# yxlllc/DDSP-SVC

Measured on AMD Instinct MI355X. Metric: audio samples/sec, CombSub 44.1kHz 256-harm hop512, higher is better.
Workload: dtype f32; 1 GPU; combsub B=32/GPU x 10 s utterances (F=862, T=441344), n_mag 256/256/256, sr 44100, hop 512, DSP path (HOT-1 + HOT-2) from resident f0 / raw controls ~N(0,1) / uniform noise, signal only; batch_per_gpu=32, frames=862, samples_per_utterance=441344, parallelism=utterance-shard x1

## Files before the change

ddsp_svc_amd/_ffi.py:

```python
import ctypes
import os
import threading

import torch

from . import build as _build

c_int, c_long, c_float, c_double, c_size_t = (ctypes.c_int, ctypes.c_long, ctypes.c_float,
                                              ctypes.c_double, ctypes.c_size_t)
P = ctypes.c_void_p

SIGNATURES = {
    "ddsp_hip_version": (c_int, []),
    "ddsp_hip_error_string": (ctypes.c_char_p, [c_int]),
    "ddsp_hip_set_tuning": (c_int, [ctypes.c_char_p, c_long]),
    "ddsp_hip_get_tuning": (c_long, [ctypes.c_char_p]),
    "ddsp_hip_window_impulse_response": (c_int, [P, c_int, P, c_long, c_int, P, P]),
    "ddsp_hip_upsample": (c_int, [P, c_int, c_int, c_int, c_int, P, P]),
    "ddsp_hip_remove_above_fmax": (c_int, [P, P, c_long, c_int, c_float, c_int, P, P]),
    "ddsp_hip_phase": (c_int, [P, P, c_int, c_int, c_int, c_double, c_int, P, P, P, P, P]),
    "ddsp_hip_ir_table_bytes": (c_size_t, [c_int]),
    "ddsp_hip_ir_table": (c_int, [c_int, P, P]),
    "ddsp_hip_allpass_response": (c_int, [P, c_long, c_long, c_int, P, P, P]),
    "ddsp_hip_impulse_response": (c_int, [P, c_long, P, c_long, c_int, c_float, c_int, P, c_long, c_int, P, P, P]),
# ... 3 lines not shown
    "ddsp_hip_allpass_backward": (c_int, [P, c_long, c_long, c_int, P, P, P, P]),
    "ddsp_hip_allpass_taps_backward": (c_int, [P, P, c_long, c_long, c_int, P, P, P, P, P]),
    "ddsp_hip_fft_convolve": (c_int, [P, c_int, P, P, P, P, c_int, c_int, c_int, c_int, c_int, P]),
    "ddsp_hip_frequency_filter_workspace_bytes": (c_size_t, [c_int, c_int, c_int]),
    "ddsp_hip_frequency_filter": (c_int, [P, P, c_long, P, c_long, c_int, P, c_int, c_int, c_int, c_int, P, P, P,
                                          c_size_t, P]),
    "ddsp_hip_fft_convolve_backward": (c_int, [P, c_int, P, P, P, P, c_int, c_int, c_int, c_int, P]),
    "ddsp_hip_sins_synth": (c_int, [P, P, P, P, c_long, P, c_long, P, c_long, P, c_int,
                                    c_int, c_int, c_int, c_double, c_int, c_int, c_int, c_int,
                                    P, P, P, P, P, P, c_size_t, c_int, P, P, ctypes.c_ulonglong, ctypes.c_ulonglong]),
    "ddsp_hip_combsub_synth": (c_int, [P, P, P, P, c_long, P, c_long, P, c_long, P, c_int,
                                       c_int, c_int, c_int, c_double, c_int, c_int, c_int, c_int,
                                       P, P, P, P, P, P, P, c_size_t, c_int, P, P, ctypes.c_ulonglong, ctypes.c_ulonglong]),
    "ddsp_hip_uniform_noise": (c_int, [ctypes.c_ulonglong, ctypes.c_ulonglong, c_int, c_long, P, P]),
    "ddsp_hip_synth_workspace_bytes": (c_size_t, [c_int, c_int, c_int, c_int]),
    "ddsp_hip_tail_layout": (c_int, [c_int, c_int, c_int, c_int, c_int, c_int, c_int, c_int, c_int, P]),
    "ddsp_hip_combsub_tail_backward_ws_bytes": (c_size_t, [c_int, c_int, c_int, c_int]),
    "ddsp_hip_combsub_tail_backward": (c_int, [P, P, c_long, P, c_long, P, c_long, P, c_int, P, P, P, c_int, c_int, c_int, c_double,
                                               c_int, P, P, P, P, P, c_size_t, P]),
    "ddsp_hip_combtooth": (c_int, [P, P, P, c_int, c_int, c_int, c_double, c_int, P, P]),
    "ddsp_hip_sinusoid_bank": (c_int, [P, P, P, P, c_long, c_int, c_int, c_int, c_int, c_double, c_int, P, P]),
    "ddsp_hip_sinusoid_bank_backward_scratch_bytes": (c_size_t, [c_int, c_int, c_int]),
    "ddsp_hip_sinusoid_bank_backward": (c_int, [P, P, P, P, c_long, P, c_int, c_int, c_int, c_int, c_double, c_int,
                                                P, P, P]),
    "ddsp_hip_fast_source": (c_int, [P, c_int, c_int, c_int, c_double, P, P, P, P]),
    "ddsp_hip_stft_filter": (c_int, [P, P, c_int, P, c_long, P, c_long, P, c_long, P, c_long, c_float, P, c_int,
                                     c_int, c_int, c_int, c_int, c_int, P, P]),
    "ddsp_hip_stft_filter_backward": (c_int, [P, P, c_int, P, c_long, P, c_long, P, c_long, P, c_long, c_float, P,
                                              c_int, c_int, c_int, P, c_int, c_int, c_int, P, P, P, P, P]),
    "ddsp_hip_combsubfast_synth": (c_int, [P, P, P, P, c_long, P, c_long, P, c_long, P, c_int, P,
# ... 177 lines not shown
```

ddsp_svc_amd/csrc/api.hip:

```cpp
#include "../../include/ddsp_hip.h"
#include "kernels.h"
#include "philox.h"
#include "splice.h"
#include "resample.h"
#include "frame_features.h"
#include "resblock.h"
#include "generator_tail.h"
#include <atomic>
#include <stdio.h>
#include <mutex>
#include <vector>
#include <stdlib.h>
#include <string.h>

using namespace ddsp;

namespace ddsp {
thread_local int t_geometry_batch = 0;
namespace {
const char* const kKnobNames[KNOB_COUNT] = {"BLK_WPS", "BLK_RUN", "BLK_PADLDS", "FFT_RUN", "STFT_WPS", "STFT_RUN",
                                            "MEL_WPS", "MEL_RUN", "FIR_MAX_SLOTS", "SINS_V1", "TAPS_GEMM", "STREAM_LAYOUT",
                                            "BLK_TURNS", "CZT_ROUNDS", "CZT_TURNS", "SINS_NOSKIP", "SMALL_PATH", "LANE_ROWS", "LANES", "FIR_BWD_DIRECT", "BWD_WPS", "TAPS_FULL",
                                            "AP_BWD_SPLIT", "SINS_SEQ", "BATCH_SPLIT"};
std::atomic<long> g_knobs[KNOB_COUNT];
std::once_flag g_knobs_once;
bool knob_is_inert(int i, long v) {
#ifdef DDSP_AB_GENERATIONS
  (void)i; (void)v;
  return false;
#else
  if (v == 0) return false;
  return i == KNOB_BLK_WPS || i == KNOB_BLK_PADLDS || (i == KNOB_SINS_V1 && v == 2);
#endif
}
void knobs_from_env() {
  for (int i = 0; i < KNOB_COUNT; ++i) {
    char name[64] = "DDSP_HIP_";
    strncat(name, kKnobNames[i], sizeof(name) - strlen(name) - 1);
// ... 48 lines not shown
  bool ok;
  Carver(void* p, size_t n) : base(static_cast<char*>(p)), size(n), used(0), ok(p != nullptr || n == 0) {}
  template <class T> T* take(size_t count) {
    size_t off = align_up(used, 256);
    size_t end = off + count * sizeof(T);
    if (end > size) { ok = false; used = end; return nullptr; }
    used = end;
    return reinterpret_cast<T*>(base + off);
  }
};

struct SynthWs {
  float *buf0, *buf1, *taps, *re, *im;
  float *taps_nz, *nzbuf;
  float *taps3;
};

struct BranchEvents {
  hipEvent_t fork = nullptr, join = nullptr, mid[2] = {nullptr, nullptr};
};

template <class T>
struct DevicePool {
  std::mutex m;
  std::vector<T*> idle[64];
  T* take(int dev) {
    std::lock_guard<std::mutex> lock(m);
    if (idle[dev].empty()) return nullptr;
    T* t = idle[dev].back();
    idle[dev].pop_back();
// ... 177 lines not shown
size_t carve_synth(Carver& c, int B, int F, int hop, int n_max, SynthWs& w) {
  const size_t BT = (size_t)B * F * hop, R = (size_t)B * F, N = 2 * (size_t)(n_max - 1);
  w.buf0 = c.take<float>(BT);
  w.buf1 = c.take<float>(BT);
  w.taps = c.take<float>(R * N);
  if (2 * R * n_max <= BT) {
    w.re = w.buf0;
    w.im = w.buf0 + R * n_max;
  } else {
    w.re = c.take<float>(R * n_max);
    w.im = c.take<float>(R * n_max);
  }
  w.taps_nz = c.take<float>(R * N);
  w.nzbuf = c.take<float>(BT);
  w.taps3 = ((long)R < kSmallRows || (n_max == 256 && hop == 512 && !fused_off())) ? c.take<float>(R * N) : nullptr;
  return align_up(c.used, 256);
}

}

extern "C" {

int ddsp_hip_version(void) { return DDSP_HIP_VERSION; }

const char* ddsp_hip_error_string(int code) {
  switch (code) {
    case 0: return "success";
    case DDSP_HIP_EINVAL: return "ddsp_hip: invalid argument (null pointer or non-positive size)";
    case DDSP_HIP_EHOP: return "ddsp_hip: hop > 2048 is not supported by the phase scan";
    case DDSP_HIP_ESHAPE: return "ddsp_hip: shape not supported by the requested kernel";
    case DDSP_HIP_EWS: return "ddsp_hip: workspace too small";
// ... 336 lines not shown
  const bool all256 = n_ap == 256 && n_harm == 256 && n_nz == 256 && !t_taps_gemm;
  float* nz = a.noise_out ? a.noise_out : w.nzbuf;
  if (w.taps3 && fused_shape_ok(R, F, hop, n_ap, n_harm, n_nz, a.fir_impl, a.gen.on != 0, true)) {
    ExciterJob exc;
    if (make_exciter_job(a.f0_frames, a.initial_phase, B, F, hop, a.sr, a.infer, a.phase0, w.buf0, &exc) != 0) return DDSP_HIP_EHOP;
    TapsJobs jobs;
    jobs.n = 0;
    const int half = taps_half_ok(F, hop, a.fir_impl) ? 1 : 0;
    int ok = launch_taps_pfa510(a.c2, a.ld2, nullptr, 0, 0, DDSP_HIP_ACT_EXP, 1.0f / 128.0f, a.t2, DDSP_HIP_MODE_HANN, nullptr, R,
                                n_nz, w.taps_nz, st, 0.f, &jobs, half);
    ok |= launch_taps_pfa510(a.c0, a.ld0, nullptr, 0, 1, DDSP_HIP_ACT_NONE, 1.0f, a.t0, DDSP_HIP_MODE_ROLL, nullptr, R, n_ap,
                             w.taps, st, 0.f, &jobs);
    ok |= launch_taps_pfa510(a.c1, a.ld1, nullptr, 0, 0, DDSP_HIP_ACT_EXP, 1.0f, a.t1, DDSP_HIP_MODE_DYNAMIC, a.f0_frames, R,
                             n_harm, w.taps3, st, (float)a.sr, &jobs);
    if (ok != 0 || launch_taps_pfa510_batch(jobs, st, &exc) != 0) return DDSP_HIP_ESHAPE;
    const FirSecond second{a.noise, a.noise_is_u01, w.taps_nz, nullptr, nz, nullptr, half};
    if (launch_fir_blk(w.buf0, 0, w.taps, nullptr, w.buf1, nullptr, B, F, hop, 2 * (n_ap - 1), st, a.gen.on ? &a.gen : nullptr, &second) < 0)
      return DDSP_HIP_ESHAPE;
    if (launch_fir(w.buf1, 0, w.taps3, nz, a.signal, a.harmonic, B, F, hop, 2 * (n_harm - 1), a.fir_impl, st) < 0)
      return DDSP_HIP_ESHAPE;
    return 0;
  }
  Branch br(st, aux_stream);
  long layout = knob(KNOB_STREAM_LAYOUT);
  if (layout != 1) layout = 4;
  if (!all256) layout = 1;
  int rc = 0;
  if (layout == 4) {
    rc = launch_combtooth(a.f0_frames, a.initial_phase, B, F, hop, a.sr, a.infer, a.phase0, w.buf0, br.aux);
    br.publish(0);
// ... 21 lines not shown

}

extern "C" {

size_t ddsp_hip_synth_workspace_bytes(int B, int F, int hop, int n_max) {
  if (B <= 0 || F <= 0 || hop <= 0 || n_max < 2) return 0;
  Carver c(nullptr, (size_t)-1);
  c.base = nullptr;
  SynthWs w;
  const LanePlan p = lane_plan(B, F);
  if (p.nsub == 1) return carve_synth(c, B, F, hop, n_max, w);
  size_t end = 0;
  for (int l = 0; l < p.slots; ++l) end = carve_synth(c, p.Bs, F, hop, n_max, w);
  return end;
}

int ddsp_hip_tail_layout(int combsub, int B, int F, int hop, int n0, int n1, int n2, int fir_impl, int in_kernel_noise,
                         long long offsets[6]) {
  if (!offsets || B <= 0 || F <= 0 || hop <= 0) return DDSP_HIP_EINVAL;
  for (int i = 0; i < 6; ++i) offsets[i] = -1;
  const TapsFormScope form;
  int n_max = n1 > n2 ? n1 : n2;
  if (combsub && n0 > n_max) n_max = n0;
  if (lane_plan(B, F).nsub > 1) return 0;
  if (!fused_shape_ok((long)B * F, F, hop, n0, n1, n2, fir_impl, in_kernel_noise != 0, combsub != 0)) return 0;
  constexpr uintptr_t kBase = 4096;
  Carver c(reinterpret_cast<void*>(kBase), (size_t)1 << 60);
  SynthWs w;
  carve_synth(c, B, F, hop, n_max, w);
// ... 143 lines not shown
  if (gen.on && !(hop == 512 && n_nz <= 257 && (fir_impl == 0 || fir_impl == 5))) return DDSP_HIP_ESHAPE;
  int n_max = n_ap > n_nz ? n_ap : n_nz;
  if (n_harm > n_max) n_max = n_harm;
  hipStream_t st = S(stream);
  const TapsFormScope form;
  const TailCall call{f0_frames, initial_phase, phase0, c_gd, ld_gd, c_harm, ld_harm, c_nz, ld_nz, noise, noise_is_u01,
                      B, F, hop, sr, infer, n_ap, n_harm, n_nz, table_ap, table_harm, table_nz, signal, harmonic_or_null,
                      noise_out_or_null, fir_impl, gen};
  const LanePlan plan = lane_plan(B, F);
  if (plan.nsub > 1) {
    const int rc = run_lanes(call, plan, ws, ws_bytes, n_max, st, aux_stream, combsub_rows);
    return rc != 0 ? rc : finish();
  }
  Carver c(ws, ws_bytes);
  SynthWs w;
  carve_synth(c, B, F, hop, n_max, w);
  if (!c.ok) return DDSP_HIP_EWS;
  const int rc = combsub_rows(call, w, st, aux_stream);
  return rc != 0 ? rc : finish();
}

size_t ddsp_hip_stft_workspace_bytes(int B, int F, int hop) {
  if (B <= 0 || F <= 0 || hop <= 0) return 0;
  return align_up((size_t)B * F * hop * sizeof(float), 256);
}

int ddsp_hip_fast_source(const float* f0_frames, int B, int F, int hop, double sr, float* rad_acc, float* phase_frames,
                         float* combtooth, void* stream) {
  if (B < 0 || F <= 0 || hop <= 0 || !(sr > 0)) return DDSP_HIP_EINVAL;
  if (B == 0) return 0;
  if (!f0_frames || !rad_acc) return DDSP_HIP_EINVAL;
  if (launch_fast_source(f0_frames, B, F, hop, sr, rad_acc, phase_frames, combtooth, S(stream)) != 0)
// ... 473 lines not shown
```

ddsp_svc_amd/csrc/fir_blk.hip:

```cpp
#include "fft_1024p.h"
#include "kernels.h"
#include "philox.h"
#include <stdlib.h>
#include <type_traits>

namespace ddsp {

using fft::cmul;

constexpr int FB_HOP = 512;

#ifdef DDSP_HIP_TIMELINE
__device__ long long* g_blk_timeline = nullptr;
__global__ void k_set_blk_timeline(long long* p) { g_blk_timeline = p; }
#define BLK_STAMP(slot) do { if (g_blk_timeline && threadIdx.x == 0 && (slot) < 32) g_blk_timeline[(long)blockIdx.x * 32 + (slot)] = (long long)wall_clock64(); } while (0)
#define BLK_STAMP_CYC(slot) do { if (g_blk_timeline && threadIdx.x == 0 && (slot) < 32) g_blk_timeline[(long)blockIdx.x * 32 + (slot)] = (long long)__builtin_readcyclecounter(); } while (0)
#define BLK_STAMP_WHERE(slot) do { if (g_blk_timeline && threadIdx.x == 0) g_blk_timeline[(long)blockIdx.x * 32 + (slot)] = ((long long)__builtin_amdgcn_s_getreg(0xF814) << 32) | (unsigned)__builtin_amdgcn_s_getreg(0xF804); } while (0)
#else
#define BLK_STAMP(slot) do { } while (0)
#define BLK_STAMP_CYC(slot) do { } while (0)
#define BLK_STAMP_WHERE(slot) do { } while (0)
#endif

struct FirBlkGeom {
// ... 222 lines not shown
    if (stamp_it) BLK_STAMP_CYC(29);
    BLK_STAMP(3 + q - q_first);
  }
}
#endif

struct FirJob {
  const float* x; int x_is_u01;
  const float* taps; const float* addend;
  float* out; float* out_plain;
  int rng;
  int taps_half;
};
struct FirJobs { FirJob j[2]; };

template <bool RNG = false, bool SEQ = false>
#ifndef DDSP_FIR_NT
#define DDSP_FIR_NT 11
#endif
#if DDSP_FIR_NT & 1
#define FB_LD_X ld_nt
#else
#define FB_LD_X ld
#endif
#if DDSP_FIR_NT & 2
#define FB_LD_T ld_nt
#else
#define FB_LD_T ld
#endif
#if DDSP_FIR_NT & 4
#define FB_ST st_nt
#else
#define FB_ST st
#endif
#if DDSP_FIR_NT & 8
#define FB_LD_A ld_nt
#else
#define FB_LD_A ld
#endif
__global__ void __launch_bounds__(128, 3) k_fir_blk6(FirJobs jobs, FirBlkGeom g, NoiseGen rng) {
  int jb = SEQ ? 0 : (int)blockIdx.y;
seq_next:
 {
  const FirJob& J = jobs.j[jb];
  const float* __restrict__ x = J.x;
  const int x_is_u01 = J.x_is_u01;
  const bool draw = RNG && J.rng != 0;
  const float* __restrict__ taps = J.taps;
  const float* __restrict__ addend = J.addend;
  float* __restrict__ out = J.out;
  float* __restrict__ out_plain = J.out_plain;
  using PL = fft::Plan1024P;
  constexpr int NF = PL::N, P = PL::P, S = 8;
  __shared__ __attribute__((aligned(16))) f32x2 ex[3][PL::WORDS];
  f32x2* const bX = ex[0];
  f32x2* const bY = ex[1];
  f32x2* const bC = ex[2];
  const int tid = threadIdx.x;
  const int b = blockIdx.x / g.runs_per_utt;
// ... 111 lines not shown
      if (m == 0) bm = own_mirror ? B0 : bm;
      a[m] = fft::add_conj(bm, a[m]);
    }
  };

  const int bw = 2 * q_first - 1;
  TapRow t1 = load_taps(bw > 0 ? bw : 0), t2 = load_taps(bw + 1);
  Blk x0 = load_blk(bw >= 0 ? bw : g.F), x1 = x0;
  typename PL::Tw tw;
  tw.init(tid);
  typename PL::Ix ix;
  ix.init(tid);
  f32x2 Hc[S];
#pragma unroll
  for (int m = 0; m < S; ++m) Hc[m] = f32x2{0.f, 0.f};
  const bool has_add = addend != nullptr, has_plain = out_plain != nullptr;
  const int turn = __builtin_amdgcn_s_getreg(0x1804) & 1;
  const int turns_mask = g.turns ? 1 : 0;
  float add[S];
#pragma unroll
  for (int i = 0; i < S; ++i) add[i] = 0.f;
  for (int q = q_first - 1; q < q_last; ++q) {
    const bool warm = q < q_first;
    if ((q + turn) & turns_mask) __builtin_amdgcn_s_setprio(1);
    else __builtin_amdgcn_s_setprio(0);
    const int b0 = 2 * q;
    f32x2 z0[S], z1[S];
#if defined(DDSP_B6_HALF_PASS_AHEAD)
    if (warm) pack_taps(t1, t2, z0);
    else pack_blk(x0, b0 < g.F, z0);
    t1 = load_taps(b0 + 3);
    t2 = load_taps(b0 + 4);
    PL::template forward_s<true, true>(z0, tw, bX, bY, ix);
// ... 22 lines not shown
#endif
    if (warm) {
      park(z0, bC);
      __syncthreads();
#pragma unroll
      for (int m = 0; m < S; ++m) z0[m] = f32x2{0.f, 0.f};
    }
    f32x2 B0;
    split_and_products(z0, z1, Hc, bC, bX, B0);
    __syncthreads();
    hermitian(z0, bX, B0);
#if defined(DDSP_B6_HALF_PASS_AHEAD)
    x0 = load_blk(b0 + 2);
    x1 = load_blk(b0 + 3);
#endif
    const int e0 = b0 * FB_HOP - 256 + tid;
    const int off_a = b0 > 0 ? 4 * e0 : BufF32::kOutOfRange;
    const int off_b = 4 * e0 + 8 * P;
    auto t_off = [&](int i) -> int { return i < 2 ? off_a + 4 * P * i : off_b + 4 * P * (i - 2); };
#if defined(DDSP_B6_HALF_PASS_AHEAD)
    if (has_add && !warm) {
#pragma unroll
      for (int i = 0; i < S; ++i) add[i] = add_buf.FB_LD_A(t_off(i));
    }
#endif
    f32x2 zt[S];
    pack_taps(t1, t2, zt);
#if !defined(DDSP_B6_HALF_PASS_AHEAD)
    t1 = load_taps(b0 + 5, pass_after);
    t2 = load_taps(b0 + 6, pass_after);
// ... 10 lines not shown
      }
#pragma unroll
      for (int i = 0; i < S; ++i) out_buf.FB_ST(fmaf(sg, d[i], add[i]), t_off(i));
      if (q == g.pairs - 1) {
#pragma unroll
        for (int m = 4; m < S; ++m) {
          const int off = t_off(4 + m);
          const float v = nsg * z0[m].y;
          if (has_plain) plain_buf.FB_ST(v, off);
          out_buf.FB_ST(v + (has_add ? add_buf.FB_LD_A(off) : 0.f), off);
        }
      }
    }
#pragma unroll
    for (int m = 0; m < 4; ++m) tail[m] = z0[4 + m].y;
#if !defined(DDSP_B6_HALF_PASS_AHEAD)
    if (has_add && q + 1 < q_last) {
      const int n0 = e0 + 2 * FB_HOP;
      const int nx_a = b0 + 2 > 0 ? 4 * n0 : BufF32::kOutOfRange, nx_b = 4 * n0 + 8 * P;
#pragma unroll
      for (int i = 0; i < S; ++i) add[i] = add_buf.FB_LD_A(i < 2 ? nx_a + 4 * P * i : nx_b + 4 * P * (i - 2));
    }
#endif
  }
 }
  if (SEQ && jb == 0) {
    jb = 1;
    __builtin_amdgcn_s_waitcnt(0);
    __syncthreads();
    goto seq_next;
// ... 9 lines not shown
#pragma unroll
  for (int m = 0; m < 4; ++m) {
    const long t = (long)bi * FB_HOP + 128 * m + threadIdx.x;
    if (t < T) out[(long)b * T + t] = q.u[m];
  }
}

int launch_uniform_noise(unsigned long long seed, unsigned long long offset, int B, long T, float* out, hipStream_t st) {
  const long wgs = (long)B * ((T + FB_HOP - 1) / FB_HOP);
  if (wgs <= 0 || wgs > 0x7fffffffL) return -1;
  hipLaunchKernelGGL(k_uniform_noise, dim3((unsigned)wgs), dim3(128), 0, st, NoiseGen{seed, offset, 1}, B, T, out);
  return 0;
}

int launch_fir_blk(const float* x, int x_is_u01, const float* taps, const float* addend, float* out, float* out_plain,
                   int B, int F, int hop, int N, hipStream_t st, const NoiseGen* noise_gen, const FirSecond* second, int taps_half) {
  if (hop != FB_HOP || N < 2 || (N & 1) || N > 512 || (long)F * hop >= (1L << 28)) return -1;
  FirBlkGeom g;
  g.F = F; g.N = N; g.T = F * hop;
  g.pairs = (F + 1) / 2;
  int wps = 3;
#ifdef DDSP_AB_GENERATIONS
  if (const long v = knob(KNOB_BLK_WPS)) { if (v >= 1) wps = (int)v; }
#endif
  const long slots = (long)wps * 2 * 256;
  const int Bg = t_geometry_batch > 0 ? t_geometry_batch : B;
  long per_utt = slots / (Bg > 0 ? Bg : 1);
  if (second && !second->seq && (long)Bg * F >= kSmallRows) per_utt = slots / (2 * (Bg > 0 ? Bg : 1));
  if (per_utt < 1) per_utt = 1;
  int run = (int)((g.pairs + per_utt - 1) / per_utt);
  if (run < 3 && (long)Bg * F >= kSmallRows) run = 3;
// ... 6 lines not shown
  if (wgs > 0x7fffffffL) return -1;
  NoiseGen rng{0ull, 0ull, 0};
  FirJobs jobs;
#ifdef DDSP_AB_GENERATIONS
  if (taps_half || (second && second->taps_half)) return -1;
#endif
  jobs.j[0] = FirJob{x, x_is_u01, taps, addend, out, out_plain, 0, taps_half};
  jobs.j[1] = jobs.j[0];
  if (second && second->seq && noise_gen && noise_gen->on) return -1;
  if (noise_gen && noise_gen->on && second) {
#ifdef DDSP_AB_GENERATIONS
    if (wps < 3) return -1;
#endif
    rng = *noise_gen;
    jobs.j[1] = FirJob{second->x, 0, second->taps, second->addend, second->out, second->out_plain, 1, second->taps_half};
    hipLaunchKernelGGL((k_fir_blk6<true>), dim3((unsigned)wgs, 2u), dim3(128), 0, st, jobs, g, rng);
    return 5;
  }
  if (noise_gen && noise_gen->on) {
    rng = *noise_gen;
    jobs.j[0].x_is_u01 = 0;
    jobs.j[0].rng = jobs.j[1].rng = 1;
#ifdef DDSP_AB_GENERATIONS
    if (wps < 3) {
      hipLaunchKernelGGL((k_fir_blk<2, true>), dim3((unsigned)wgs), dim3(128), 0, st, x, 0, taps, addend, out, out_plain, g, rng);
      return 5;
    }
#endif
    hipLaunchKernelGGL((k_fir_blk6<true>), dim3((unsigned)wgs), dim3(128), 0, st, jobs, g, rng);
    return 5;
  }
  if (second && second->seq) {
    if (wps < 3 || (noise_gen && noise_gen->on)) return -1;
    jobs.j[1] = FirJob{second->x, second->x_is_u01, second->taps, second->addend, second->out, second->out_plain, 0, second->taps_half};
    hipLaunchKernelGGL((k_fir_blk6<false, true>), dim3((unsigned)wgs), dim3(128), 0, st, jobs, g, rng);
    return 5;
  }
  if (second && wps >= 3) {
    jobs.j[1] = FirJob{second->x, second->x_is_u01, second->taps, second->addend, second->out, second->out_plain, 0, second->taps_half};
    hipLaunchKernelGGL((k_fir_blk6<false>), dim3((unsigned)wgs, 2u), dim3(128), 0, st, jobs, g, rng);
    return 5;
  }
  if (second) return -1;
#ifdef DDSP_AB_GENERATIONS
  size_t pad = 0;
  if (const long v = knob(KNOB_BLK_PADLDS)) { if (v > 0) pad = (size_t)v; }
  if (wps < 3 || pad != 0) {
    hipLaunchKernelGGL((k_fir_blk<2, false>), dim3((unsigned)wgs), dim3(128), pad, st, x, x_is_u01, taps, addend, out, out_plain, g, rng);
    return 5;
  }
#endif
  hipLaunchKernelGGL((k_fir_blk6<false>), dim3((unsigned)wgs), dim3(128), 0, st, jobs, g, rng);
  return 5;
}

}

#ifdef DDSP_HIP_TIMELINE
extern "C" int ddsp_hip_debug_set_blk_timeline(long long* p, void* stream) {
  hipLaunchKernelGGL(ddsp::k_set_blk_timeline, dim3(1), dim3(1), 0, (hipStream_t)stream, p);
  return (int)hipGetLastError();
}
#endif
```

ddsp_svc_amd/csrc/kernels.h:

```cpp
#pragma once
#include <hip/hip_runtime.h>
#include <stddef.h>
#include "ddsp_common.h"
#include "tuning.h"

namespace ddsp {
extern thread_local int t_geometry_batch;
int spl_for_hop(int hop);
void launch_upsample(const float* sig, int B, int F, int C, int hop, float* out, hipStream_t st);
void launch_remove_above_fmax(const float* amps, const float* pitch, long rows, int H, float fmax, int level_start,
                              float* out, hipStream_t st);
int launch_phase(const float* f0_frames, const float* initial_phase, int B, int F, int hop, double sr, int infer,
                 double* frame_sums, double* phase0, float* phase_frames, float* x_or_null, hipStream_t st);
int launch_combtooth(const float* f0_frames, const float* initial_phase, int B, int F, int hop, double sr, int infer,
                     const double* phase0, float* out, hipStream_t st);
int launch_sins_bank(const float* f0_frames, const float* initial_phase, const float* c_amp, long ld_amp, int B, int F,
                     int hop, int H, double sr, int infer, const double* phase0, float* out, hipStream_t st);
size_t sins_bank_bwd_scratch_floats(int B, int F, int H);
int launch_sins_bank_bwd(const float* f0_frames, const float* initial_phase, const float* c_amp, long ld_amp,
                         const float* grad_out, int B, int F, int hop, int H, double sr, int infer, const double* phase0,
                         float* scratch, float* d_c, hipStream_t st);
size_t ir_table_floats(int n);
void launch_ir_table(int n, float* table, hipStream_t st);
void launch_allpass_response(const float* c, long ld, long rows, int n, float* re, float* im, hipStream_t st);
// ... 45 lines not shown
struct TapsBwdJobs { TapsBwdJob j[3]; int n; };
int launch_taps_pfa510_bwd_jobs(const TapsBwdJobs& jobs, const float* table, long rows, hipStream_t st);
void launch_window_taps(const float* in, int mode, const float* half_width, long rows, int N, float* out, hipStream_t st);
void launch_allpass_backward(const float* c, long ld, long rows, int n, const float* d_re, const float* d_im, float* d_c,
                             hipStream_t st);
size_t fir_mfma_lds_bytes(int F, int hop, int N, int waves);
struct NoiseGen;
int launch_fir(const float* x, int x_is_u01, const float* taps, const float* addend, float* out, float* out_plain,
               int B, int F, int hop, int N, int impl, hipStream_t st, const NoiseGen* noise_gen = nullptr);
int launch_uniform_noise(unsigned long long seed, unsigned long long offset, int B, long T, float* out, hipStream_t st);
int launch_fir_fft(const float* x, int x_is_u01, const float* taps, const float* addend, float* out, float* out_plain,
                   int B, int F, int hop, int N, hipStream_t st);
struct FirSecond { const float* x; int x_is_u01; const float* taps; const float* addend; float* out; float* out_plain; int taps_half; int seq = 0; };
int launch_fir_blk(const float* x, int x_is_u01, const float* taps, const float* addend, float* out, float* out_plain,
                   int B, int F, int hop, int N, hipStream_t st, const NoiseGen* noise_gen = nullptr,
                   const FirSecond* second = nullptr, int taps_half = 0);
struct FirBwdSecond { const float* x; int x_is_u01; const float* grad_out; float* d_taps; };
int launch_fir_blk_bwd(const float* x, int x_is_u01, const float* taps, const float* grad_out, float* d_x, float* d_taps,
                       int B, int F, int hop, int N, hipStream_t st, const FirBwdSecond* second = nullptr);
int launch_fir_fft_bwd(const float* x, int x_is_u01, const float* taps, const float* grad_out, float* d_x, float* d_taps,
                       int B, int F, int hop, int N, hipStream_t st);
int launch_fir_bwd_direct(const float* x, int x_is_u01, const float* taps, const float* grad_out, float* d_x, float* d_taps,
                          int B, int F, int hop, int N, hipStream_t st);
int launch_fast_source(const float* f0_frames, int B, int F, int hop, double sr, float* rad_acc, float* phase_frames,
                       float* combtooth, hipStream_t st);
int launch_fast_combtooth(const float* f0_frames, const float* rad_acc, int B, int F, int hop, double sr, float* out,
                          hipStream_t st);
int launch_stft_filter(const float* exc, const float* noise, int noise_is_u01, const float* c_hmag, long ld_hm,
                       const float* c_hphase, long ld_hp, const float* c_nmag, long ld_nm, const float* c_nphase,
                       long ld_np, float noise_scale, const float* window, int win, int reflect, int normalize, int B,
                       int F, int hop, float* out, hipStream_t st,
// ... 65 lines not shown
```

ddsp_svc_amd/csrc/tuning.h:

```cpp
#pragma once

namespace ddsp {

enum Knob {
  KNOB_BLK_WPS = 0, KNOB_BLK_RUN, KNOB_BLK_PADLDS, KNOB_FFT_RUN, KNOB_STFT_WPS, KNOB_STFT_RUN, KNOB_MEL_WPS,
  KNOB_MEL_RUN, KNOB_FIR_MAX_SLOTS, KNOB_SINS_V1, KNOB_TAPS_GEMM, KNOB_STREAM_LAYOUT, KNOB_BLK_TURNS, KNOB_CZT_ROUNDS, KNOB_CZT_TURNS,
  KNOB_SINS_NOSKIP, KNOB_SMALL_PATH, KNOB_LANE_ROWS, KNOB_LANES, KNOB_FIR_BWD_DIRECT, KNOB_BWD_WPS, KNOB_TAPS_FULL,
  KNOB_AP_BWD_SPLIT, KNOB_SINS_SEQ, KNOB_BATCH_SPLIT,
  KNOB_COUNT
};

constexpr long kSmallRows = 4096;

long knob(Knob k);
int knob_set(const char* name, long v);
long knob_get(const char* name);

constexpr long kMaxGridYZ = 65535;
inline long batch_split() {
  const long v = knob(KNOB_BATCH_SPLIT);
  return v >= 1 && v <= kMaxGridYZ ? v : kMaxGridYZ;
}

}
// ... 1 lines not shown
```

ddsp_svc_amd/synth.py:

```python
import os
from dataclasses import dataclass
from typing import Optional

import torch

from . import _ffi
from ._ffi import ptr
from .core import _f32c, ir_table

_EARLY_JOIN = os.environ.get("DDSP_HIP_TRAIN_EARLY_JOIN", "0") == "1"
_TRAIN_COMPOSED = os.environ.get("DDSP_HIP_TRAIN_COMPOSED", "0") == "1"


@dataclass
class PhaseState:
    phase0: torch.Tensor
    phase_frames: torch.Tensor
    initial_phase: Optional[torch.Tensor]
    infer: bool
    x: Optional[torch.Tensor] = None


def _rows(t, n):
    if t.dtype != torch.float32:
# ... 43 lines not shown


def sinusoid_bank(f0_frames, state: PhaseState, amplitudes_ctrl, sampling_rate, block_size):
    f0 = _f32c(f0_frames.reshape(f0_frames.shape[0], -1))
    B, F = f0.shape
    hop = int(block_size)
    H = amplitudes_ctrl.shape[-1]
    c, ld = _rows(amplitudes_ctrl, H)
    out = torch.empty(B, F * hop, dtype=torch.float32, device=f0.device)
    _ffi.check(_ffi.lib().ddsp_hip_sinusoid_bank(ptr(f0), ptr(state.initial_phase), ptr(state.phase0), ptr(c), ld,
                                                 B, F, hop, H, float(sampling_rate), int(state.infer), ptr(out),
                                                 _ffi.stream_of(f0)))
    return out


def _workspace(B, F, hop, n_max, device):
    need = _ffi.lib().ddsp_hip_synth_workspace_bytes(B, F, hop, n_max)
    return torch.empty(need, dtype=torch.uint8, device=device), need


def _outputs(B, T, device, want_components):
    signal = torch.empty(B, T, dtype=torch.float32, device=device)
    if want_components:
        return signal, torch.empty_like(signal), torch.empty_like(signal)
    return signal, None, None


def uniform_noise(B, T, seed, offset, device):
    out = torch.empty(B, T, dtype=torch.float32, device=device)
    _ffi.check_device(out)
    _ffi.check(_ffi.lib().ddsp_hip_uniform_noise(int(seed), int(offset), B, T, ptr(out), _ffi.stream_of(out)))
    return out
# ... 364 lines not shown
        if lay is not None:
            return CombSubTailFunction.apply(f0, state, group_delay, harmonic_magnitude, noise_magnitude,
                                             _f32c(noise.reshape(B, -1)), noise_is_u01, sampling_rate, int(block_size), lay)
        return _combsub_synth_train(f0_frames, state, group_delay, harmonic_magnitude, noise_magnitude, noise,
                                    sampling_rate, block_size, noise_is_u01)
    f0 = _f32c(f0_frames.reshape(f0_frames.shape[0], -1))
    B, F = f0.shape
    hop = int(block_size)
    T = F * hop
    n_ap, n_h, n_nz = group_delay.shape[-1], harmonic_magnitude.shape[-1], noise_magnitude.shape[-1]
    cg, ldg = _rows(group_delay, n_ap)
    ch, ldh = _rows(harmonic_magnitude, n_h)
    cn, ldn = _rows(noise_magnitude, n_nz)
    dev = f0.device
    nz, is_u01, seed, offset = _noise_arg(noise, noise_seed, noise_offset, noise_is_u01, B, T, hop, n_nz, fir_impl, dev)
    ws, need = _workspace(B, F, hop, max(n_ap, n_h, n_nz), dev)
    signal, harm, nzo = _outputs(B, T, dev, want_components)
    if signal_out is not None:
        if tuple(signal_out.shape) != (B, T) or signal_out.dtype != torch.float32 or signal_out.device != dev or not signal_out.is_contiguous():
            raise ValueError("signal_out must be a contiguous float32 [%d, %d] tensor on %s" % (B, T, dev))
        signal = signal_out
    _ffi.check(_ffi.lib().ddsp_hip_combsub_synth(
        ptr(f0), ptr(state.initial_phase), ptr(state.phase0), ptr(cg), ldg, ptr(ch), ldh, ptr(cn), ldn,
        ptr(nz), int(is_u01), B, F, hop, float(sampling_rate), int(state.infer), n_ap, n_h, n_nz,
        ptr(ir_table(n_ap, dev)), ptr(ir_table(n_h, dev)), ptr(ir_table(n_nz, dev)),
        ptr(signal), ptr(harm), ptr(nzo), ptr(ws), need, int(fir_impl), _ffi.stream_of(f0), _ffi.aux_stream_of(f0, B * F),
        seed, offset))
    return signal, harm, nzo


class StreamingCombSub:

    def __init__(self, B, F, n_mag_allpass, n_mag_harmonic, n_mag_noise, sampling_rate, block_size, device, infer=True,
                 want_components=False):
        self.B, self.F, self.hop, self.sr, self.infer = int(B), int(F), int(block_size), float(sampling_rate), bool(infer)
        self.n = (int(n_mag_allpass), int(n_mag_harmonic), int(n_mag_noise))
        dev = torch.device(device)
        T = self.F * self.hop
        self._sums = torch.empty(B, F, dtype=torch.float64, device=dev)
        self.state = PhaseState(torch.empty(B, F, dtype=torch.float64, device=dev), torch.empty(B, F, 1, dtype=torch.float32, device=dev),
                                None, self.infer)
        self._ws, self._need = _workspace(B, F, self.hop, max(self.n), dev)
        self.signal, self.harmonic, self.noise = _outputs(B, T, dev, want_components)
        self._tables = tuple(ir_table(n, dev) for n in self.n)
        self._lib = _ffi.lib()
        _ffi.check_device(self.signal)
        self._dev = self.signal.device
        self._stream = _ffi.stream_of(self.signal)

    def _check(self, t, shape, what):
        if t.device != self._dev or t.dtype != torch.float32 or tuple(t.shape) != shape or t.stride(-1) != 1:
            raise ValueError("StreamingCombSub: %s must be a float32 %s tensor on %s with a contiguous last dimension (got %s %s on %s, "
                             "strides %s)" % (what, shape, self._dev, t.dtype, tuple(t.shape), t.device, tuple(t.stride())))

    def _check_ctrl(self, t, n, what):
        self._check(t, (self.B, self.F, n), what)
        if t.stride(1) < n or (self.B > 1 and t.stride(0) != self.F * t.stride(1)):
# ... 244 lines not shown
```

include/ddsp_hip.h:

```cpp
#ifndef DDSP_HIP_H
#define DDSP_HIP_H
#include <stddef.h>

#ifdef __cplusplus
extern "C" {
#endif

#define DDSP_HIP_VERSION 165

#define DDSP_HIP_EINVAL   (-1)
#define DDSP_HIP_EHOP     (-2)
#define DDSP_HIP_ESHAPE   (-3)
#define DDSP_HIP_EWS      (-4)

#define DDSP_HIP_MODE_ROLL    0
#define DDSP_HIP_MODE_HANN    1
#define DDSP_HIP_MODE_DYNAMIC 2

#define DDSP_HIP_ACT_NONE 0
#define DDSP_HIP_ACT_EXP  1

#define DDSP_HIP_FIR_AUTO   0
#define DDSP_HIP_FIR_SIMPLE 1
#define DDSP_HIP_FIR_MFMA   2
// ... 61 lines not shown
                        float* signal, float* harmonic_or_null, float* noise_out_or_null,
                        void* ws, size_t ws_bytes, int fir_impl, void* stream, void* aux_stream,
                        unsigned long long noise_seed, unsigned long long noise_offset);

int ddsp_hip_combsub_synth(const float* f0_frames, const float* initial_phase, const double* phase0,
                           const float* c_gd, long ld_gd, const float* c_harm, long ld_harm,
                           const float* c_nz, long ld_nz, const float* noise, int noise_is_u01,
                           int B, int F, int hop, double sr, int infer, int n_ap, int n_harm, int n_nz,
                           const float* table_ap, const float* table_harm, const float* table_nz,
                           float* signal, float* harmonic_or_null, float* noise_out_or_null,
                           void* ws, size_t ws_bytes, int fir_impl, void* stream, void* aux_stream,
                           unsigned long long noise_seed, unsigned long long noise_offset);


size_t ddsp_hip_synth_workspace_bytes(int B, int F, int hop, int n_max);

int ddsp_hip_tail_layout(int combsub, int B, int F, int hop, int n0, int n1, int n2, int fir_impl, int in_kernel_noise,
                         long long offsets[6]);

size_t ddsp_hip_combsub_tail_backward_ws_bytes(int B, int F, int hop, int n_mag);
int ddsp_hip_combsub_tail_backward(const float* f0_frames, const float* c_gd, long ld_gd, const float* c_harm, long ld_harm,
                                   const float* c_nz, long ld_nz, const float* noise, int noise_is_u01, const void* fwd_ws,
                                   const float* g_harm, const float* g_noise, int B, int F, int hop, double sr, int n_mag,
                                   const float* table, float* d_gd, float* d_harm, float* d_nz, void* ws, size_t ws_bytes,
                                   void* stream);

int ddsp_hip_combtooth(const float* f0_frames, const float* initial_phase, const double* phase0, int B, int F,
                       int hop, double sr, int infer, float* out, void* stream);
int ddsp_hip_sinusoid_bank(const float* f0_frames, const float* initial_phase, const double* phase0,
                           const float* c_amp, long ld_amp, int B, int F, int hop, int H, double sr, int infer,
// ... 141 lines not shown
```

Baseline: 48.71 billion samples/s.

## Sum noise branch in spectral domain instead of time-domain addend

When only the mixed signal is requested, the noise FIR pass writes its frequency-domain block spectra to a new workspace region instead of running the inverse transform and writing time-domain noise. The harmonic FIR pass then adds those spectra before its own inverse transform. This removes one inverse FFT pass and one full-length time-domain buffer write and read. In exchange it needs extra workspace, new kernel template variants, and a knob to disable it.

```diff
diff --git a/ddsp_svc_amd/_ffi.py b/ddsp_svc_amd/_ffi.py
--- a/ddsp_svc_amd/_ffi.py
+++ b/ddsp_svc_amd/_ffi.py
@@ -41,6 +41,7 @@
                                        P, P, P, P, P, P, P, c_size_t, c_int, P, P, ctypes.c_ulonglong, ctypes.c_ulonglong]),
     "ddsp_hip_uniform_noise": (c_int, [ctypes.c_ulonglong, ctypes.c_ulonglong, c_int, c_long, P, P]),
     "ddsp_hip_synth_workspace_bytes": (c_size_t, [c_int, c_int, c_int, c_int]),
+    "ddsp_hip_synth_signal_workspace_bytes": (c_size_t, [c_int, c_int, c_int, c_int]),
     "ddsp_hip_tail_layout": (c_int, [c_int, c_int, c_int, c_int, c_int, c_int, c_int, c_int, c_int, P]),
     "ddsp_hip_combsub_tail_backward_ws_bytes": (c_size_t, [c_int, c_int, c_int, c_int]),
     "ddsp_hip_combsub_tail_backward": (c_int, [P, P, c_long, P, c_long, P, c_long, P, c_int, P, P, P, c_int, c_int, c_int, c_double,
diff --git a/ddsp_svc_amd/csrc/api.hip b/ddsp_svc_amd/csrc/api.hip
--- a/ddsp_svc_amd/csrc/api.hip
+++ b/ddsp_svc_amd/csrc/api.hip
@@ -21,7 +21,7 @@
 const char* const kKnobNames[KNOB_COUNT] = {"BLK_WPS", "BLK_RUN", "BLK_PADLDS", "FFT_RUN", "STFT_WPS", "STFT_RUN",
                                             "MEL_WPS", "MEL_RUN", "FIR_MAX_SLOTS", "SINS_V1", "TAPS_GEMM", "STREAM_LAYOUT",
                                             "BLK_TURNS", "CZT_ROUNDS", "CZT_TURNS", "SINS_NOSKIP", "SMALL_PATH", "LANE_ROWS", "LANES", "FIR_BWD_DIRECT", "BWD_WPS", "TAPS_FULL",
-                                            "AP_BWD_SPLIT", "SINS_SEQ", "BATCH_SPLIT"};
+                                            "AP_BWD_SPLIT", "SINS_SEQ", "BATCH_SPLIT", "SPECTRAL_SUM"};
 std::atomic<long> g_knobs[KNOB_COUNT];
 std::once_flag g_knobs_once;
 bool knob_is_inert(int i, long v) {
@@ -100,6 +100,7 @@
   float *buf0, *buf1, *taps, *re, *im;
   float *taps_nz, *nzbuf;
   float *taps3;
+  float *spec;
 };
 
 struct BranchEvents {
@@ -307,7 +308,12 @@
   w.taps_nz = c.take<float>(R * N);
   w.nzbuf = c.take<float>(BT);
   w.taps3 = ((long)R < kSmallRows || (n_max == 256 && hop == 512 && !fused_off())) ? c.take<float>(R * N) : nullptr;
+  w.spec = nullptr;
   return align_up(c.used, 256);
+}
+
+size_t spec_floats(int B, int F, int hop, int n_max) {
+  return n_max == 256 && hop == 512 ? (size_t)B * (size_t)((F + 1) / 2) * 2048 : 0;
 }
 
 }
@@ -674,6 +680,15 @@
     ok |= launch_taps_pfa510(a.c1, a.ld1, nullptr, 0, 0, DDSP_HIP_ACT_EXP, 1.0f, a.t1, DDSP_HIP_MODE_DYNAMIC, a.f0_frames, R,
                              n_harm, w.taps3, st, (float)a.sr, &jobs);
     if (ok != 0 || launch_taps_pfa510_batch(jobs, st, &exc) != 0) return DDSP_HIP_ESHAPE;
+    const long ss = knob(KNOB_SPECTRAL_SUM);
+    if (w.spec && !a.harmonic && !a.noise_out && ss != 1 && (R >= kSmallRows || ss == 2) && t_geometry_batch == 0) {
+      const FirSecond second{a.noise, a.noise_is_u01, w.taps_nz, nullptr, w.spec, nullptr, half};
+      if (launch_fir_blk(w.buf0, 0, w.taps, nullptr, w.buf1, nullptr, B, F, hop, 2 * (n_ap - 1), st, a.gen.on ? &a.gen : nullptr, &second, 0, 1) < 0)
+        return DDSP_HIP_ESHAPE;
+      if (launch_fir_blk(w.buf1, 0, w.taps3, w.spec, a.signal, nullptr, B, F, hop, 2 * (n_harm - 1), st, nullptr, nullptr, 0, 2) < 0)
+        return DDSP_HIP_ESHAPE;
+      return 0;
+    }
     const FirSecond second{a.noise, a.noise_is_u01, w.taps_nz, nullptr, nz, nullptr, half};
     if (launch_fir_blk(w.buf0, 0, w.taps, nullptr, w.buf1, nullptr, B, F, hop, 2 * (n_ap - 1), st, a.gen.on ? &a.gen : nullptr, &second) < 0)
       return DDSP_HIP_ESHAPE;
@@ -725,6 +740,12 @@
   size_t end = 0;
   for (int l = 0; l < p.slots; ++l) end = carve_synth(c, p.Bs, F, hop, n_max, w);
   return end;
+}
+
+size_t ddsp_hip_synth_signal_workspace_bytes(int B, int F, int hop, int n_max) {
+  const size_t base = ddsp_hip_synth_workspace_bytes(B, F, hop, n_max);
+  if (base == 0 || lane_plan(B, F).nsub > 1) return base;
+  return align_up(base + spec_floats(B, F, hop, n_max) * sizeof(float), 256);
 }
 
 int ddsp_hip_tail_layout(int combsub, int B, int F, int hop, int n0, int n1, int n2, int fir_impl, int in_kernel_noise,
@@ -898,8 +919,10 @@
   }
   Carver c(ws, ws_bytes);
   SynthWs w;
-  carve_synth(c, B, F, hop, n_max, w);
+  const size_t base = carve_synth(c, B, F, hop, n_max, w);
   if (!c.ok) return DDSP_HIP_EWS;
+  const size_t sf = spec_floats(B, F, hop, n_max);
+  if (sf != 0 && ws_bytes >= base && ws_bytes - base >= sf * sizeof(float)) w.spec = reinterpret_cast<float*>(static_cast<char*>(ws) + base);
   const int rc = combsub_rows(call, w, st, aux_stream);
   return rc != 0 ? rc : finish();
 }
diff --git a/ddsp_svc_amd/csrc/fir_blk.hip b/ddsp_svc_amd/csrc/fir_blk.hip
--- a/ddsp_svc_amd/csrc/fir_blk.hip
+++ b/ddsp_svc_amd/csrc/fir_blk.hip
@@ -260,7 +260,7 @@
 };
 struct FirJobs { FirJob j[2]; };
 
-template <bool RNG = false, bool SEQ = false>
+template <bool RNG = false, bool SEQ = false, int SPEC = 0>
 #ifndef DDSP_FIR_NT
 #define DDSP_FIR_NT 11
 #endif
@@ -289,6 +289,8 @@
 seq_next:
  {
   const FirJob& J = jobs.j[jb];
+  const bool spec_out = SPEC == 1 && jb == 1;
+  constexpr bool SPEC_IN = SPEC == 2;
   const float* __restrict__ x = J.x;
   const int x_is_u01 = J.x_is_u01;
   const bool draw = RNG && J.rng != 0;
@@ -430,9 +432,22 @@
   f32x2 Hc[S];
 #pragma unroll
   for (int m = 0; m < S; ++m) Hc[m] = f32x2{0.f, 0.f};
-  const bool has_add = addend != nullptr, has_plain = out_plain != nullptr;
+  const bool has_add = !SPEC_IN && addend != nullptr, has_plain = out_plain != nullptr;
   const int turn = __builtin_amdgcn_s_getreg(0x1804) & 1;
   const int turns_mask = g.turns ? 1 : 0;
+  auto spec_planes = [&](const float* base, int q, bool live, BufF32& re, BufF32& im) {
+    const float* p = base + ((long)bu * g.pairs + (live ? q : 0)) * (2 * NF);
+    re = BufF32::make(p, live ? NF : 0);
+    im = BufF32::make(p + NF, live ? NF : 0);
+  };
+  f32x2 sp[S];
+  auto load_spec = [&](int q, bool live) {
+    BufF32 re, im;
+    spec_planes(addend, q, live, re, im);
+#pragma unroll
+    for (int m = 0; m < S; ++m) sp[m] = f32x2{re.FB_LD_A(tid4 + 4 * P * m), im.FB_LD_A(tid4 + 4 * P * m)};
+  };
+  if (SPEC_IN) load_spec(q_first - 1, q_first > 0);
   float add[S];
 #pragma unroll
   for (int i = 0; i < S; ++i) add[i] = 0.f;
@@ -485,6 +500,30 @@
     x0 = load_blk(b0 + 2);
     x1 = load_blk(b0 + 3);
 #endif
+    if (SPEC_IN) {
+#pragma unroll
+      for (int m = 0; m < S; ++m) z0[m] = z0[m] + sp[m];
+    }
+    if (spec_out) {
+      if (!warm) {
+        BufF32 re, im;
+        spec_planes(out, q, true, re, im);
+#pragma unroll
+        for (int m = 0; m < S; ++m) {
+          re.FB_ST(z0[m].x, tid4 + 4 * P * m);
+          im.FB_ST(z0[m].y, tid4 + 4 * P * m);
+        }
+      }
+      f32x2 zs[S];
+      pack_taps(t1, t2, zs);
+#if !defined(DDSP_B6_HALF_PASS_AHEAD)
+      t1 = load_taps(b0 + 5, pass_after);
+      t2 = load_taps(b0 + 6, pass_after);
+#endif
+      PL::template forward_s<true, true>(zs, tw, bC, bY, ix);
+      park(zs, bC);
+      continue;
+    }
     const int e0 = b0 * FB_HOP - 256 + tid;
     const int off_a = b0 > 0 ? 4 * e0 : BufF32::kOutOfRange;
     const int off_b = 4 * e0 + 8 * P;
@@ -525,6 +564,7 @@
     }
 #pragma unroll
     for (int m = 0; m < 4; ++m) tail[m] = z0[4 + m].y;
+    if (SPEC_IN && q + 1 < q_last) load_spec(q + 1, true);
 #if !defined(DDSP_B6_HALF_PASS_AHEAD)
     if (has_add && q + 1 < q_last) {
       const int n0 = e0 + 2 * FB_HOP;
@@ -564,7 +604,10 @@
 }
 
 int launch_fir_blk(const float* x, int x_is_u01, const float* taps, const float* addend, float* out, float* out_plain,
-                   int B, int F, int hop, int N, hipStream_t st, const NoiseGen* noise_gen, const FirSecond* second, int taps_half) {
+                   int B, int F, int hop, int N, hipStream_t st, const NoiseGen* noise_gen, const FirSecond* second, int taps_half,
+                   int spec) {
+  if (spec != 0 && !(spec == 1 ? second && !second->seq && !second->addend && !second->out_plain
+                               : spec == 2 && !second && addend && !(noise_gen && noise_gen->on))) return -1;
   if (hop != FB_HOP || N < 2 || (N & 1) || N > 512 || (long)F * hop >= (1L << 28)) return -1;
   FirBlkGeom g;
   g.F = F; g.N = N; g.T = F * hop;
@@ -601,9 +644,11 @@
 #endif
     rng = *noise_gen;
     jobs.j[1] = FirJob{second->x, 0, second->taps, second->addend, second->out, second->out_plain, 1, second->taps_half};
-    hipLaunchKernelGGL((k_fir_blk6<true>), dim3((unsigned)wgs, 2u), dim3(128), 0, st, jobs, g, rng);
+    if (spec == 1) hipLaunchKernelGGL((k_fir_blk6<true, false, 1>), dim3((unsigned)wgs, 2u), dim3(128), 0, st, jobs, g, rng);
+    else hipLaunchKernelGGL((k_fir_blk6<true>), dim3((unsigned)wgs, 2u), dim3(128), 0, st, jobs, g, rng);
     return 5;
   }
+  if (spec != 0 && wps < 3) return -1;
   if (noise_gen && noise_gen->on) {
     rng = *noise_gen;
     jobs.j[0].x_is_u01 = 0;
@@ -625,7 +670,8 @@
   }
   if (second && wps >= 3) {
     jobs.j[1] = FirJob{second->x, second->x_is_u01, second->taps, second->addend, second->out, second->out_plain, 0, second->taps_half};
-    hipLaunchKernelGGL((k_fir_blk6<false>), dim3((unsigned)wgs, 2u), dim3(128), 0, st, jobs, g, rng);
+    if (spec == 1) hipLaunchKernelGGL((k_fir_blk6<false, false, 1>), dim3((unsigned)wgs, 2u), dim3(128), 0, st, jobs, g, rng);
+    else hipLaunchKernelGGL((k_fir_blk6<false>), dim3((unsigned)wgs, 2u), dim3(128), 0, st, jobs, g, rng);
     return 5;
   }
   if (second) return -1;
@@ -637,7 +683,8 @@
     return 5;
   }
 #endif
-  hipLaunchKernelGGL((k_fir_blk6<false>), dim3((unsigned)wgs), dim3(128), 0, st, jobs, g, rng);
+  if (spec == 2) hipLaunchKernelGGL((k_fir_blk6<false, false, 2>), dim3((unsigned)wgs), dim3(128), 0, st, jobs, g, rng);
+  else hipLaunchKernelGGL((k_fir_blk6<false>), dim3((unsigned)wgs), dim3(128), 0, st, jobs, g, rng);
   return 5;
 }
 
diff --git a/ddsp_svc_amd/csrc/kernels.h b/ddsp_svc_amd/csrc/kernels.h
--- a/ddsp_svc_amd/csrc/kernels.h
+++ b/ddsp_svc_amd/csrc/kernels.h
@@ -83,7 +83,7 @@
 struct FirSecond { const float* x; int x_is_u01; const float* taps; const float* addend; float* out; float* out_plain; int taps_half; int seq = 0; };
 int launch_fir_blk(const float* x, int x_is_u01, const float* taps, const float* addend, float* out, float* out_plain,
                    int B, int F, int hop, int N, hipStream_t st, const NoiseGen* noise_gen = nullptr,
-                   const FirSecond* second = nullptr, int taps_half = 0);
+                   const FirSecond* second = nullptr, int taps_half = 0, int spec = 0);
 struct FirBwdSecond { const float* x; int x_is_u01; const float* grad_out; float* d_taps; };
 int launch_fir_blk_bwd(const float* x, int x_is_u01, const float* taps, const float* grad_out, float* d_x, float* d_taps,
                        int B, int F, int hop, int N, hipStream_t st, const FirBwdSecond* second = nullptr);
diff --git a/ddsp_svc_amd/csrc/tuning.h b/ddsp_svc_amd/csrc/tuning.h
--- a/ddsp_svc_amd/csrc/tuning.h
+++ b/ddsp_svc_amd/csrc/tuning.h
@@ -6,7 +6,7 @@
   KNOB_BLK_WPS = 0, KNOB_BLK_RUN, KNOB_BLK_PADLDS, KNOB_FFT_RUN, KNOB_STFT_WPS, KNOB_STFT_RUN, KNOB_MEL_WPS,
   KNOB_MEL_RUN, KNOB_FIR_MAX_SLOTS, KNOB_SINS_V1, KNOB_TAPS_GEMM, KNOB_STREAM_LAYOUT, KNOB_BLK_TURNS, KNOB_CZT_ROUNDS, KNOB_CZT_TURNS,
   KNOB_SINS_NOSKIP, KNOB_SMALL_PATH, KNOB_LANE_ROWS, KNOB_LANES, KNOB_FIR_BWD_DIRECT, KNOB_BWD_WPS, KNOB_TAPS_FULL,
-  KNOB_AP_BWD_SPLIT, KNOB_SINS_SEQ, KNOB_BATCH_SPLIT,
+  KNOB_AP_BWD_SPLIT, KNOB_SINS_SEQ, KNOB_BATCH_SPLIT, KNOB_SPECTRAL_SUM,
   KNOB_COUNT
 };
 
diff --git a/ddsp_svc_amd/synth.py b/ddsp_svc_amd/synth.py
--- a/ddsp_svc_amd/synth.py
+++ b/ddsp_svc_amd/synth.py
@@ -81,8 +81,9 @@
     return out
 
 
-def _workspace(B, F, hop, n_max, device):
-    need = _ffi.lib().ddsp_hip_synth_workspace_bytes(B, F, hop, n_max)
+def _workspace(B, F, hop, n_max, device, signal_only=False):
+    lib = _ffi.lib()
+    need = (lib.ddsp_hip_synth_signal_workspace_bytes if signal_only else lib.ddsp_hip_synth_workspace_bytes)(B, F, hop, n_max)
     return torch.empty(need, dtype=torch.uint8, device=device), need
 
 
@@ -477,7 +478,7 @@
     cn, ldn = _rows(noise_magnitude, n_nz)
     dev = f0.device
     nz, is_u01, seed, offset = _noise_arg(noise, noise_seed, noise_offset, noise_is_u01, B, T, hop, n_nz, fir_impl, dev)
-    ws, need = _workspace(B, F, hop, max(n_ap, n_h, n_nz), dev)
+    ws, need = _workspace(B, F, hop, max(n_ap, n_h, n_nz), dev, signal_only=not want_components)
     signal, harm, nzo = _outputs(B, T, dev, want_components)
     if signal_out is not None:
         if tuple(signal_out.shape) != (B, T) or signal_out.dtype != torch.float32 or signal_out.device != dev or not signal_out.is_contiguous():
@@ -503,7 +504,7 @@
         self._sums = torch.empty(B, F, dtype=torch.float64, device=dev)
         self.state = PhaseState(torch.empty(B, F, dtype=torch.float64, device=dev), torch.empty(B, F, 1, dtype=torch.float32, device=dev),
                                 None, self.infer)
-        self._ws, self._need = _workspace(B, F, self.hop, max(self.n), dev)
+        self._ws, self._need = _workspace(B, F, self.hop, max(self.n), dev, signal_only=not want_components)
         self.signal, self.harmonic, self.noise = _outputs(B, T, dev, want_components)
         self._tables = tuple(ir_table(n, dev) for n in self.n)
         self._lib = _ffi.lib()
diff --git a/include/ddsp_hip.h b/include/ddsp_hip.h
--- a/include/ddsp_hip.h
+++ b/include/ddsp_hip.h
@@ -99,6 +99,7 @@
 
 
 size_t ddsp_hip_synth_workspace_bytes(int B, int F, int hop, int n_max);
+size_t ddsp_hip_synth_signal_workspace_bytes(int B, int F, int hop, int n_max);
 
 int ddsp_hip_tail_layout(int combsub, int B, int F, int hop, int n0, int n1, int n2, int fir_impl, int in_kernel_noise,
                          long long offsets[6]);
```

Result: no change. 48.82 billion samples/s, median of 2 (+0.2%).
